# milos-agathon/vulkan-forge

Measured on AMD Instinct MI355X. Metric: Mpix/s terrain shade (grid=4096, 4096x4096), higher is better.
Workload: dtype f32

## Files before the change

### include/vf_hip.h

```cpp
#ifndef VF_HIP_H
#define VF_HIP_H

#include <stddef.h>
#include <stdint.h>

#ifdef __cplusplus
extern "C" {
#endif

#define VF_OK 0
#define VF_ERR_NO_DEVICE (-1)
#define VF_ERR_HIP (-2)
#define VF_ERR_INVALID (-3)
#define VF_ERR_NOMEM (-4)

typedef struct vf_ctx vf_ctx;
typedef struct vf_terrain vf_terrain;

typedef struct vf_device_info {
    char name[256];
    char arch[64];
    int32_t device_ordinal;
    int32_t compute_units;
    int32_t wavefront_size;
// ... 71 lines not shown
int vf_terrain_add_points(vf_terrain *t, const float *xyz, uint32_t n, const float *size_px, const uint8_t *rgba, float default_size,
                          const uint8_t default_rgba[4], int shape, int drape, uint32_t *layer_id);
int vf_terrain_add_lines(vf_terrain *t, const float *xyz, const uint32_t *path_offsets, uint32_t npaths, float width_px,
                         const uint8_t rgba[4], int cap, int drape, uint32_t *layer_id);
int vf_terrain_clear_overlays(vf_terrain *t);
int vf_terrain_add_polygons(vf_terrain *t, const float *xyz, const uint32_t *ring_offsets, uint32_t nrings, const uint32_t *feature_offsets,
                            uint32_t nfeatures, const uint8_t *fill_rgba, const uint8_t default_fill[4], const uint8_t line_rgba[4],
                            float line_width_px, int drape, uint32_t *layer_id);
#define VF_OCCLUSION_DEPTH_BIAS 1e-2f
int vf_terrain_set_layer_occlusion(vf_terrain *t, uint32_t layer_id, int occlude, float depth_bias);
int vf_terrain_set_layer_haze(vf_terrain *t, uint32_t layer_id, int on);
int vf_terrain_layer_haze(vf_terrain *t, uint32_t layer_id, int *on);
#define VF_JOIN_ROUND 0
#define VF_JOIN_NONE 1
int vf_terrain_add_contours(vf_terrain *t, const float *levels, uint32_t nlevels, float width_px, const uint8_t rgba[4], float lift, int join,
                            int occlude, float depth_bias, uint32_t *layer_id, uint32_t *nsegments);
int vf_terrain_height_bounds(vf_terrain *t, float *lo, float *hi);
int vf_terrain_layer_primitive_count(vf_terrain *t, uint32_t layer_id, uint32_t *count);

int vf_terrain_read_rgba(vf_terrain *t, uint8_t *dst, uint32_t y0, uint32_t rows);
int vf_host_alloc(size_t bytes, void **host);
void vf_host_free(void *host);
int vf_terrain_read_png_scanlines(vf_terrain *t, const uint8_t **host_scanlines, size_t *nbytes);
int vf_terrain_read_visibility(vf_terrain *t, uint32_t *dst);

int vf_terrain_enable_timing(vf_terrain *t, int enable);
int vf_terrain_timings(vf_terrain *t, vf_timings *out);
int vf_terrain_frame_times(vf_terrain *t, float *tile_ms, float *period_ms, uint32_t max_frames, uint32_t *count);
int vf_terrain_debug_item_stats(vf_terrain *t, uint32_t *dst, uint32_t max_items, uint32_t *count);
#define VF_BAND_SLOTS 8u
int vf_terrain_debug_band_masks(vf_terrain *t, uint32_t *recs, uint64_t *masks, int32_t *xy, uint32_t max_blocks, uint32_t *count);
int vf_terrain_debug_set_plan_feedback(vf_terrain *t, const uint32_t *tile_ticks, const uint8_t *strips_log2, const uint32_t *piece_ticks,
                                       uint32_t ntiles);
#define VF_PLAN_FIRST        1u
#define VF_PLAN_FRESH        2u
#define VF_PLAN_MOTION_MAP   4u
#define VF_PLAN_DILATE       8u
#define VF_PLAN_QUEUED_AHEAD 16u
#define VF_PLAN_GEOMETRY_REUSED 32u
#define VF_PLAN_TILE_LISTS   64u
int vf_terrain_debug_plan_mode(const vf_terrain *t, uint32_t *mode);
typedef struct vf_tile_list_info { uint32_t built, used, tiles_listed, tiles_fallback, entries, capacity, units_asked, reserved; } vf_tile_list_info;
int vf_terrain_debug_tile_lists(vf_terrain *t, vf_tile_list_info *out);
int vf_terrain_debug_set_tile_list_capacity(vf_terrain *t, uint32_t units);
int vf_terrain_debug_phase_cycles(vf_terrain *t, uint64_t *dst, uint32_t n);

int vf_grid_generate(vf_ctx *ctx, uint32_t nx, uint32_t nz, float dx, float dy,
                     float *xy, float *uv, uint32_t *idx);
int vf_grid_generate_device(vf_ctx *ctx, uint32_t nx, uint32_t nz, float dx, float dy,
                            float *dev_xy, float *dev_uv, uint32_t *dev_idx, void *stream);

int vf_triangle_render(vf_ctx *ctx, uint32_t width, uint32_t height, uint8_t *rgba_host);

typedef struct vf_dem vf_dem;
int vf_dem_create(vf_ctx *ctx, vf_dem **out);
void vf_dem_destroy(vf_dem *d);
int vf_dem_set_heights_f32(vf_dem *d, const float *host, uint32_t w, uint32_t h, float exaggeration);
int vf_dem_set_heights_f64(vf_dem *d, const double *host, uint32_t w, uint32_t h, float exaggeration);
int vf_dem_stats(vf_dem *d, float out[4]);
int vf_dem_percentile_range(vf_dem *d, float *p1, float *p99);
int vf_dem_normalize(vf_dem *d, int mode, float lo, float hi, float eps);
int vf_dem_upload_height(vf_dem *d);
int vf_dem_texture_size(const vf_dem *d, uint32_t *w, uint32_t *h);
int vf_dem_read_patch(vf_dem *d, uint32_t x, uint32_t y, uint32_t w, uint32_t h, float *dst);

int vf_stitch_bands_device(vf_ctx *ctx, const void *dev_gathered, void *dev_image, uint32_t width,
// ... 221 lines not shown
```

### vulkan_forge_amd/cabi.py

```python
from __future__ import annotations

import ctypes as C
import os

import numpy as np

_HERE = os.path.dirname(os.path.abspath(__file__))
DEFAULT_LIB = os.environ.get("VF_HIP_LIB") or os.path.join(_HERE, "libvf_hip.so")

VF_OK, VF_ERR_NO_DEVICE, VF_ERR_HIP, VF_ERR_INVALID, VF_ERR_NOMEM = 0, -1, -2, -3, -4
VF_DRAPE_SIZE_MAX, VF_DRAPE_NEAREST, VF_DRAPE_LINEAR = 16384, 0, 1
VF_DRAPE_MIP_BIAS_MAX, VF_DRAPE_MIP_LEVELS_MAX = 16.0, 15
VF_DRAPE_ANISOTROPY_MAX = 16
VF_SUPERSAMPLE_MAX = 4
VF_PLAN_FIRST, VF_PLAN_FRESH, VF_PLAN_MOTION_MAP, VF_PLAN_DILATE, VF_PLAN_QUEUED_AHEAD = 1, 2, 4, 8, 16
VF_PLAN_TILE_LISTS = 64
VF_PLAN_GEOMETRY_REUSED = 32

SYMBOLS = [
    "vf_last_error", "vf_device_count", "vf_device_query", "vf_ctx_create", "vf_ctx_destroy", "vf_ctx_device_info", "vf_ctx_stream",
    "vf_terrain_create", "vf_terrain_destroy", "vf_terrain_set_uniforms", "vf_terrain_set_height",
    "vf_terrain_set_height_device", "vf_terrain_set_shade_mode", "vf_terrain_set_shade_precision", "vf_terrain_set_raster_groups", "vf_terrain_raster_groups", "vf_terrain_set_shard", "vf_terrain_local_rows", "vf_terrain_set_tile_shard",
    "vf_terrain_local_tiles", "vf_terrain_read_tiles", "vf_tile_layout", "vf_terrain_tile_times", "vf_balance_stripes", "vf_tile_layout_register_map", "vf_terrain_set_output_device",
    "vf_terrain_rgba_device", "vf_terrain_render", "vf_terrain_render_batch", "vf_terrain_render_batch_host", "vf_terrain_sync",
    "vf_terrain_add_points", "vf_terrain_add_lines", "vf_terrain_add_polygons", "vf_terrain_set_layer_occlusion", "vf_terrain_set_layer_haze", "vf_terrain_layer_haze", "vf_terrain_add_contours", "vf_terrain_height_bounds", "vf_terrain_layer_primitive_count", "vf_terrain_clear_overlays", "vf_terrain_read_rgba", "vf_terrain_read_png_scanlines", "vf_terrain_read_visibility",
    "vf_terrain_enable_timing", "vf_terrain_timings", "vf_terrain_frame_times", "vf_terrain_debug_item_stats", "vf_terrain_debug_band_masks", "vf_terrain_debug_set_plan_feedback", "vf_terrain_debug_plan_mode", "vf_terrain_debug_tile_lists", "vf_terrain_debug_set_tile_list_capacity", "vf_terrain_debug_phase_cycles", "vf_grid_generate", "vf_grid_generate_device", "vf_triangle_render",
    "vf_stitch_bands_device", "vf_stitch_tiles_device",
    "vf_dist_available", "vf_dist_version", "vf_dist_unique_id", "vf_dist_comm_init", "vf_dist_comm_destroy", "vf_dist_gather_tiles", "vf_dist_gather_bands", "vf_dist_exchange_bands",
    "vf_terrain_debug_fragment_stage", "vf_host_alloc", "vf_host_free",
    "vf_terrain_gbuffer_device", "vf_terrain_read_gbuffer", "vf_terrain_pick", "vf_terrain_debug_gbuffer_stage",
    "vf_terrain_set_shadows", "vf_terrain_read_shadow_field", "vf_terrain_shadow_field_device", "vf_terrain_debug_shadow_stage",
    "vf_terrain_debug_shadow_scans",
    "vf_terrain_set_ambient", "vf_terrain_read_sky_view_field", "vf_terrain_sky_view_field_device", "vf_terrain_debug_ambient_stage",
    "vf_terrain_debug_ambient_scans",
    "vf_terrain_set_drape", "vf_terrain_set_drape_device", "vf_terrain_clear_drape", "vf_terrain_drape_info", "vf_terrain_debug_drape_stage",
    "vf_terrain_set_drape_mips", "vf_terrain_drape_mip_info", "vf_terrain_read_drape_level", "vf_terrain_debug_drape_mip_build",
    "vf_terrain_set_drape_anisotropy", "vf_terrain_drape_anisotropy",
    "vf_terrain_set_viewshed", "vf_terrain_read_viewshed_field", "vf_terrain_viewshed_field_device", "vf_terrain_viewshed_info",
    "vf_terrain_debug_viewshed_stage", "vf_terrain_debug_viewshed_scans",
    "vf_terrain_set_cumulative_viewshed", "vf_terrain_read_cumulative_viewshed_field", "vf_terrain_cumulative_viewshed_field_device",
    "vf_terrain_cumulative_viewshed_info", "vf_terrain_read_cumulative_viewshed_vertices", "vf_terrain_debug_cumulative_viewshed_batch",
    "vf_terrain_debug_cumulative_viewshed_scans", "vf_terrain_debug_cumulative_viewshed_stage",
    "vf_terrain_set_sun_exposure", "vf_terrain_clear_sun_exposure", "vf_terrain_read_sun_exposure_field", "vf_terrain_sun_exposure_field_device",
    "vf_terrain_sun_exposure_info", "vf_terrain_debug_sun_exposure_batch", "vf_terrain_debug_sun_exposure_scans",
    "vf_terrain_debug_sun_exposure_stage",
    "vf_terrain_create_supersampled", "vf_terrain_supersampling", "vf_terrain_read_samples", "vf_terrain_samples_device",
    "vf_terrain_debug_resolve_stage",
    "vf_terrain_set_haze", "vf_terrain_clear_haze", "vf_terrain_haze_info", "vf_terrain_read_haze_opacity", "vf_terrain_haze_opacity_device",
    "vf_terrain_debug_haze_stage",
    "vf_terrain_set_flood", "vf_terrain_clear_flood", "vf_terrain_read_flood_field", "vf_terrain_flood_field_device", "vf_terrain_flood_info",
    "vf_terrain_read_flood_seeds", "vf_terrain_debug_flood_scans", "vf_terrain_debug_flood_group", "vf_terrain_debug_flood_stage",
    "vf_terrain_set_spill", "vf_terrain_clear_spill", "vf_terrain_read_spill_field", "vf_terrain_spill_field_device", "vf_terrain_read_sink_depth",
    "vf_terrain_spill_info", "vf_terrain_read_spill_seeds", "vf_terrain_debug_spill_scans", "vf_terrain_debug_spill_group",
    "vf_terrain_debug_spill_stage",
    "vf_dem_create", "vf_dem_destroy", "vf_dem_set_heights_f32", "vf_dem_set_heights_f64", "vf_dem_stats",
    "vf_dem_percentile_range", "vf_dem_normalize", "vf_dem_upload_height", "vf_dem_texture_size", "vf_dem_read_patch",
]


# ... 65 lines not shown
    "vf_terrain_set_raster_groups": (_i, [_vp, _i]),
    "vf_terrain_raster_groups": (_i, [_vp, C.POINTER(_i), _vp]),
    "vf_terrain_set_shard": (_i, [_vp, _u32, _u32, _u32]),
    "vf_terrain_local_rows": (_i, [_vp, C.POINTER(_u32)]),
    "vf_terrain_set_tile_shard": (_i, [_vp, _u32, _u32, _u32]),
    "vf_terrain_add_points": (_i, [_vp, _vp, _u32, _vp, _vp, _f, _vp, _i, _i, C.POINTER(_u32)]),
    "vf_terrain_add_lines": (_i, [_vp, _vp, _vp, _u32, _f, _vp, _i, _i, C.POINTER(_u32)]),
    "vf_terrain_add_polygons": (_i, [_vp, _vp, _vp, _u32, _vp, _u32, _vp, _vp, _vp, _f, _i, C.POINTER(_u32)]),
    "vf_terrain_set_layer_occlusion": (_i, [_vp, _u32, _i, _f]),
    "vf_terrain_set_layer_haze": (_i, [_vp, _u32, _i]),
    "vf_terrain_layer_haze": (_i, [_vp, _u32, C.POINTER(C.c_int)]),
    "vf_terrain_add_contours": (_i, [_vp, _vp, _u32, _f, _vp, _f, _i, _i, _f, C.POINTER(_u32), C.POINTER(_u32)]),
    "vf_terrain_height_bounds": (_i, [_vp, C.POINTER(_f), C.POINTER(_f)]),
    "vf_terrain_layer_primitive_count": (_i, [_vp, _u32, C.POINTER(_u32)]),
    "vf_terrain_clear_overlays": (_i, [_vp]),
    "vf_terrain_local_tiles": (_i, [_vp, C.POINTER(_u32)]),
    "vf_terrain_read_tiles": (_i, [_vp, _vp, _u32, _u32]),
    "vf_tile_layout": (_i, [_u32, _u32, _u32, _u32, _u32, _vp, _u32, C.POINTER(_u32)]),
    "vf_terrain_set_output_device": (_i, [_vp, _vp]),
    "vf_terrain_rgba_device": (_i, [_vp, C.POINTER(_vp)]),
    "vf_terrain_render": (_i, [_vp, _vp]),
    "vf_terrain_render_batch": (_i, [_vp, _vp, _u32, _vp, _vp]),
    "vf_terrain_render_batch_host": (_i, [_vp, _vp, _u32, _vp]),
    "vf_terrain_sync": (_i, [_vp]),
    "vf_terrain_read_rgba": (_i, [_vp, _vp, _u32, _u32]),
    "vf_terrain_read_png_scanlines": (_i, [_vp, C.POINTER(_vp), C.POINTER(C.c_size_t)]),
    "vf_terrain_read_visibility": (_i, [_vp, _vp]),
    "vf_terrain_enable_timing": (_i, [_vp, _i]),
    "vf_terrain_timings": (_i, [_vp, C.POINTER(Timings)]),
    "vf_terrain_frame_times": (_i, [_vp, _vp, _vp, _u32, C.POINTER(_u32)]),
    "vf_terrain_debug_item_stats": (_i, [_vp, _vp, _u32, C.POINTER(_u32)]),
    "vf_terrain_debug_band_masks": (_i, [_vp, _vp, _vp, _vp, _u32, C.POINTER(_u32)]),
    "vf_terrain_debug_set_plan_feedback": (_i, [_vp, _vp, _vp, _vp, _u32]),
    "vf_terrain_debug_plan_mode": (_i, [_vp, C.POINTER(_u32)]),
    "vf_terrain_debug_tile_lists": (_i, [_vp, _vp]),
    "vf_terrain_debug_set_tile_list_capacity": (_i, [_vp, _u32]),
    "vf_terrain_debug_phase_cycles": (_i, [_vp, _vp, _u32]),
    "vf_terrain_tile_times": (_i, [_vp, _vp, _u32, C.POINTER(_u32)]),
    "vf_balance_stripes": (_i, [_vp, _u32, _u32, _vp]),
    "vf_tile_layout_register_map": (_i, [_vp, _u32, _u32, _u32, C.POINTER(_u32)]),
    "vf_host_alloc": (_i, [C.c_size_t, C.POINTER(_vp)]),
    "vf_host_free": (None, [_vp]),
    "vf_grid_generate": (_i, [_vp, _u32, _u32, _f, _f, _vp, _vp, _vp]),
    "vf_grid_generate_device": (_i, [_vp, _u32, _u32, _f, _f, _vp, _vp, _vp, _vp]),
    "vf_triangle_render": (_i, [_vp, _u32, _u32, _vp]),
    "vf_stitch_bands_device": (_i, [_vp, _vp, _vp, _u32, _u32, _u32, _u32, _vp]),
    "vf_stitch_tiles_device": (_i, [_vp, _vp, _vp, _u32, _u32, _u32, _u32, _u32, _vp]),
    "vf_dist_available": (_i, []),
    "vf_dist_version": (_i, [C.POINTER(_i)]),
    "vf_dist_unique_id": (_i, [_vp]),
    "vf_dist_comm_init": (_i, [_vp, _vp, _i, _i, C.POINTER(_vp)]),
    "vf_dist_comm_destroy": (None, [_vp]),
    "vf_dist_gather_tiles": (_i, [_vp, _vp, _i, _vp, _u32, _vp]),
    "vf_dist_gather_bands": (_i, [_vp, _vp, _i, _vp, _vp]),
    "vf_dist_exchange_bands": (_i, [_vp, _vp, _i, _vp, _vp]),
    "vf_terrain_debug_fragment_stage": (_i, [_vp, _u32, C.POINTER(FragmentTiming)]),
    "vf_terrain_gbuffer_device": (_i, [_vp, _vp, _vp, _vp, _vp, _vp]),
    "vf_terrain_read_gbuffer": (_i, [_vp, _vp, _vp, _vp, _vp]),
    "vf_terrain_pick": (_i, [_vp, _vp, _u32, _vp]),
    "vf_terrain_debug_gbuffer_stage": (_i, [_vp, _u32, _u32, C.POINTER(_f)]),
    "vf_terrain_set_shadows": (_i, [_vp, _i, _f, _f, _f]),
    "vf_terrain_read_shadow_field": (_i, [_vp, _vp]),
    "vf_terrain_shadow_field_device": (_i, [_vp, _vp, _vp]),
    "vf_terrain_debug_shadow_stage": (_i, [_vp, _u32, C.POINTER(_f)]),
    "vf_terrain_debug_shadow_scans": (_i, [_vp, C.POINTER(_u32)]),
    "vf_terrain_set_ambient": (_i, [_vp, _i, _f, _f, _u32, _vp]),
# ... 768 lines not shown
        a = _u32()
        self._check(self.lib.vf_terrain_drape_anisotropy(self.t, C.byref(a)))
        return a.value

    def enable_timing(self, on=True, stats=True, sampled=False):
        self._check(self.lib.vf_terrain_enable_timing(self.t, (1 if stats else (3 if sampled else 2)) if on else 0))

    def item_stats(self):
        cap = self.timings()["tiles"] + 2048
        out = np.zeros((cap, 4), np.uint32)
        n = _u32()
        self._check(self.lib.vf_terrain_debug_item_stats(self.t, out.ctypes.data, cap, C.byref(n)))
        return out[:n.value]

    def band_masks(self):
        nb = (self.grid - 1 + 7) // 8
        n = nb * nb
        recs, masks, xy = np.zeros((n, 8), np.uint32), np.zeros((n, 8, 2), np.uint64), np.zeros((n, 81, 2), np.int32)
        got = _u32()
        self._check(self.lib.vf_terrain_debug_band_masks(self.t, recs.ctypes.data, masks.ctypes.data, xy.ctypes.data, n, C.byref(got)))
        assert got.value == n
        wide = recs[:, 4:8].copy().view(np.uint64)
        return dict(box=recs[:, 0:2].copy().view(np.int16), flags=recs[:, 2].copy(), count=recs[:, 3].copy(),
                    alive_even=wide[:, 0].copy(), alive_odd=wide[:, 1].copy(), masks=masks, xy=xy)

    def set_plan_feedback(self, tile_ticks, strips_log2=None, piece_ticks=None):
        ticks = np.ascontiguousarray(tile_ticks, dtype=np.uint32).reshape(-1)
        n = len(ticks)
        lg = np.zeros(n, np.uint8) if strips_log2 is None else np.ascontiguousarray(strips_log2, dtype=np.uint8).reshape(n)
        pieces = None if piece_ticks is None else np.ascontiguousarray(piece_ticks, dtype=np.uint32).reshape(n, 64)
        self._check(self.lib.vf_terrain_debug_set_plan_feedback(self.t, ticks.ctypes.data, lg.ctypes.data,
                                                                None if pieces is None else pieces.ctypes.data, n))

    def plan_mode(self, geometry=False):
        m = _u32()
        self._check(self.lib.vf_terrain_debug_plan_mode(self.t, C.byref(m)))
        return m.value if geometry else m.value & ~(VF_PLAN_GEOMETRY_REUSED | VF_PLAN_TILE_LISTS)

    def tile_lists(self):
        w = (_u32 * 8)()
        self._check(self.lib.vf_terrain_debug_tile_lists(self.t, C.addressof(w)))
        names = ("built", "used", "tiles_listed", "tiles_fallback", "entries", "capacity", "units_asked")
        d = dict(zip(names, (int(v) for v in w)))
        d["built"], d["used"] = bool(d["built"]), bool(d["used"])
        return d

    def set_tile_list_capacity(self, units=0xFFFFFFFF):
        self._check(self.lib.vf_terrain_debug_set_tile_list_capacity(self.t, units))

    def geometry_reused(self):
        return bool(self.plan_mode(geometry=True) & VF_PLAN_GEOMETRY_REUSED)

    def tile_stats(self):
        it = self.item_stats()
        out = np.zeros((self.timings()["tiles"], 3), np.uint32)
        tile = it[:, 0] & 0xFFFFF
        np.add.at(out[:, 0], tile, it[:, 1])
        np.maximum.at(out[:, 1], tile, it[:, 2])
        np.maximum.at(out[:, 2], tile, it[:, 3])
        return out

    def phase_cycles(self):
        out = np.zeros(40, np.uint64)
        self._check(self.lib.vf_terrain_debug_phase_cycles(self.t, out.ctypes.data, 40))
        return out

# ... 76 lines not shown
```

### vulkan_forge_amd/csrc/vf_device.h

```cpp
#pragma once
#include <hip/hip_runtime.h>
#include <stdint.h>

#define VF_RESERVE_VGPR(n) asm volatile("" ::: "v" #n)

namespace vf {

constexpr int kBlockCells = 8;
constexpr int kBlockVerts = kBlockCells + 1;
constexpr int kTileW = 64, kTileH = 64;
constexpr uint32_t kSplitQuantumX4 = 7;
#ifndef VF_TILE_MIN_WAVES
#define VF_TILE_MIN_WAVES 5
#endif
#ifndef VF_DIAG_ITEM
#define VF_DIAG_ITEM 0
#endif
constexpr int kDiagItem = VF_DIAG_ITEM;
constexpr int kMaxTileCols = 256;
constexpr int kPhaseSlots = 40;
constexpr int kTileThreads = 1024;
constexpr int kFastExtent = 1 << 24;

constexpr uint32_t F_NEAR = 1u, F_FAR = 2u, F_BAD = 4u, F_NOSNAP = 8u;

struct FrameParams {
    float view[16];
    float proj[16];
    float spacing, exag;
    float h_range, exposure;
    float Lx, Ly, Lz;
    float hw, hh;
    float step;
    uint32_t n, nm1;
    uint32_t nb;
    uint32_t W, H;
    uint32_t ntx, nty;
    uint32_t tw, th;
    uint32_t rank, nranks, band_shift, band_h;
    uint32_t local_rows;
    uint32_t shard_tiles;
    uint32_t skew;
    uint32_t stripe_shift;
    const uint32_t *tile_map;
    const uint8_t *stripe_owner;
    uint32_t clear_rgba;
    uint32_t shade_mode;
    const float *tex;
    float inv2hr;
    uint32_t div_m, div_s;
};
// ... 266 lines not shown
```

### vulkan_forge_amd/csrc/vf_hip.hip

```cpp
#include "../../include/vf_hip.h"
#include "vf_kernels.h"
#include "vf_overlay.h"
#include "vf_gbuffer.h"
#include "vf_shadow.h"
#include "vf_ambient.h"
#include "vf_drape.h"
#include "vf_relight.h"
#include "vf_viewshed.h"
#include "vf_cumulative_viewshed.h"
#include "vf_sun_exposure.h"
#include "vf_resolve.h"
#include "vf_haze.h"
#include "vf_overlay_haze.h"
#include "vf_flood.h"
#include "vf_spill.h"
#include "vf_line_loop.h"

#include <algorithm>
#include <cmath>
#include <vector>
#include <cstddef>
#include <cstdio>
#include <cstring>
#include <cstdlib>
// ... 4075 lines not shown
    *count = (uint32_t)nb;
    return VF_OK;
}

int vf_terrain_debug_set_plan_feedback(vf_terrain *t, const uint32_t *tile_ticks, const uint8_t *strips_log2, const uint32_t *piece_ticks,
                                       uint32_t ntiles)
{
    if (!t || !tile_ticks || !strips_log2) return fail(VF_ERR_INVALID, "NULL argument");
    if (ntiles != t->local_tiles) return fail(VF_ERR_INVALID, "ntiles must be the handle's local tiles");
    for (uint32_t k = 0; k < ntiles; ++k) if (strips_log2[k] > 4u) return fail(VF_ERR_INVALID, "strips_log2 must be 0 .. 4");
    if (t->cursor.frames_since_reset < vf_terrain::kPlanStates)
        return fail(VF_ERR_INVALID, "the handle's first frames are planned from the static estimate: render two frames first");
    for (const auto &S : t->ps) if (!S.slab) return fail(VF_ERR_INVALID, "a plan state has not been used yet: render two frames first");
    VF_HIP_TRY(hipSetDevice(t->ctx->device));
    VF_HIP_TRY(wait_frame(t));
    VF_HIP_TRY(sync_sides(t));
    VF_HIP_TRY(drop_preplan(t));
    VF_HIP_TRY(wait_frame(t));
    VF_HIP_TRY(sync_sides(t));
    if (!ntiles) return VF_OK;
    const size_t all_tiles = (size_t)t->ntx * t->nty;
    std::vector<uint32_t> pieces((size_t)ntiles * 64u, 0u), flags(ntiles);
    if (piece_ticks) std::memcpy(pieces.data(), piece_ticks, pieces.size() * sizeof(uint32_t));
    for (auto &S : t->ps) {
        VF_HIP_TRY(hipMemcpy(S.feedback, tile_ticks, (size_t)ntiles * sizeof(uint32_t), hipMemcpyHostToDevice));
        VF_HIP_TRY(hipMemcpy(S.feedback + all_tiles + 1u, pieces.data(), pieces.size() * sizeof(uint32_t), hipMemcpyHostToDevice));
        VF_HIP_TRY(hipMemcpy(flags.data(), S.background, (size_t)ntiles * sizeof(uint32_t), hipMemcpyDeviceToHost));
        for (uint32_t k = 0; k < ntiles; ++k) flags[k] = (flags[k] & 0xFFu) | ((uint32_t)strips_log2[k] << 8);
        VF_HIP_TRY(hipMemcpy(S.background, flags.data(), (size_t)ntiles * sizeof(uint32_t), hipMemcpyHostToDevice));
    }
    return VF_OK;
}

int vf_terrain_debug_plan_mode(const vf_terrain *t, uint32_t *mode)
{
    if (!t || !mode) return fail(VF_ERR_INVALID, "NULL argument");
    if (!t->rendered) return fail(VF_ERR_INVALID, "nothing rendered yet");
    *mode = t->last_plan_mode;
    return VF_OK;
}

int vf_terrain_debug_tile_lists(vf_terrain *t, vf_tile_list_info *out)
{
    if (!t || !out) return fail(VF_ERR_INVALID, "NULL argument");
    if (!t->rendered) return fail(VF_ERR_INVALID, "nothing rendered yet");
    VF_HIP_TRY(hipSetDevice(t->ctx->device));
    std::memset(out, 0, sizeof *out);
    const vf_terrain::PlanState &S = t->ps[t->last_set];
    out->used = (t->last_plan_mode & VF_PLAN_TILE_LISTS) ? 1u : 0u;
    out->built = lists_valid(t, S) ? 1u : 0u;
    if (!out->built && !out->used) return VF_OK;
    VF_HIP_TRY(hipEventSynchronize(S.listed));
    uint32_t ctl[8];
    VF_HIP_TRY(hipMemcpy(ctl, S.tl_ctl, sizeof ctl, hipMemcpyDeviceToHost));
    out->tiles_listed = ctl[2]; out->tiles_fallback = ctl[3]; out->entries = ctl[4];
    out->capacity = S.tl_cap;
    const unsigned long long asked = (unsigned long long)ctl[0] | ((unsigned long long)ctl[1] << 32);
    out->units_asked = asked > 0xFFFFFFFFull ? 0xFFFFFFFFu : (uint32_t)asked;
    return VF_OK;
}

int vf_terrain_debug_set_tile_list_capacity(vf_terrain *t, uint32_t units)
{
    if (!t) return fail(VF_ERR_INVALID, "NULL argument");
    VF_HIP_TRY(hipSetDevice(t->ctx->device));
    VF_HIP_TRY(wait_frame(t));
// ... 1031 lines not shown
```

### vulkan_forge_amd/csrc/vf_kernels.h

```cpp
#pragma once
#include "vf_device.h"
#include "vf_raster.h"

namespace vf {

__global__ void k_axis_tables(uint32_t n, uint32_t tw, uint32_t th, float *xs, float *sinx, float *cosz,
                              int32_t *txi, int32_t *tyj)
{
    uint32_t i = blockIdx.x * blockDim.x + threadIdx.x;
    if (i >= n) return;
    const float scale = 1.5f;
    const float nm1f = (float)n - 1.0f;
    const float step = (2.0f * scale) / nm1f;
    float x = -scale + (float)i * step;
    float uvc = (float)i / nm1f;
    xs[i] = x;
    sinx[i] = det_sin(x * 1.3f);
    cosz[i] = det_cos(x * 1.1f);
    int tx = (int)floorf(uvc * (float)tw), ty = (int)floorf(uvc * (float)th);
    txi[i] = min(max(tx, 0), (int)tw - 1);
    tyj[i] = min(max(ty, 0), (int)th - 1);
}

__global__ __launch_bounds__(64) void k_height_blocks(uint32_t n, uint32_t nb, uint32_t tw, AxisTables A,
// ... 889 lines not shown
        if ((uint32_t)colbits) atomicOr(&colfin[2 * lane], (uint32_t)colbits);
        if ((uint32_t)(colbits >> 32)) atomicOr(&colfin[2 * lane + 1], (uint32_t)(colbits >> 32));
    }
    return nfinal;
}

struct TilePlace { uint32_t tx; size_t out_base; uint32_t out_stride; };
__device__ __forceinline__ TilePlace tile_rect(const FrameParams &P, uint32_t tile, int32_t &px_lo, int32_t &px_hi, int32_t &py_lo, int32_t &py_hi)
{
    TilePlace tp;
    if (P.shard_tiles) {
        const uint32_t m = P.tile_map[tile];
        tp.tx = m & 0xFFFFu;
        py_lo = (int32_t)((m >> 16) * kTileH);
        tp.out_base = (size_t)tile * (kTileW * kTileH);
        tp.out_stride = kTileW;
    } else {
        tp.tx = tile % P.ntx;
        const uint32_t lty = tile / P.ntx;
        py_lo = (int32_t)global_row(P, lty * kTileH);
        tp.out_base = (size_t)lty * kTileH * P.W + (size_t)tp.tx * kTileW;
        tp.out_stride = P.W;
    }
    px_lo = (int32_t)(tp.tx * kTileW); px_hi = min(px_lo + kTileW, (int32_t)P.W) - 1;
    py_hi = min(py_lo + kTileH, (int32_t)P.H) - 1;
    return tp;
}

constexpr uint32_t kSplitBudget = 2048;
__device__ __forceinline__ uint32_t work_tile(uint32_t code) { return code & 0xFFFFFu; }
__device__ __forceinline__ uint32_t work_part(uint32_t code) { return (code >> 20) & 15u; }
__device__ __forceinline__ uint32_t work_slice(uint32_t code) { return (code >> 27) & 3u; }
__device__ __forceinline__ uint32_t work_lg_slices(uint32_t code) { return (code >> 29) & 3u; }
__device__ __forceinline__ void work_strip(uint32_t code, int32_t &px_lo, int32_t &px_hi)
{
    const uint32_t lg = (code >> 24) & 7u, part = (code >> 20) & 15u;
    const int32_t w = kTileW >> lg;
    const int32_t lo = px_lo + (int32_t)part * w;
    px_hi = min(px_hi, lo + w - 1);
    px_lo = lo;
}


__device__ __forceinline__ uint32_t tile_reach(const FrameParams &P, const PixelBox *__restrict__ row_boxes, const uint32_t *__restrict__ rc_lo,
                                               const uint32_t *__restrict__ rc_hi, uint32_t tcol, int32_t py_lo, int32_t py_hi,
                                               uint32_t *s_hits, uint32_t *s_est)
{
    if (threadIdx.x == 0) { *s_hits = 0; *s_est = 0; }
    __syncthreads();
    uint32_t hits = 0, est = 0;
    for (uint32_t r = threadIdx.x; r < P.nb; r += 256) {
        const PixelBox rr = row_boxes[r];
        const uint32_t lo = rc_lo[tcol * P.nb + r], hi = rc_hi[tcol * P.nb + r];
        if (lo < hi && rr.x0 <= rr.x1 && rr.y1 >= py_lo && rr.y0 <= py_hi) { ++hits; est += hi - lo; }
    }
    for (int o = 32; o > 0; o >>= 1) { hits += __shfl_xor(hits, o); est += __shfl_xor(est, o); }
    if ((threadIdx.x & 63u) == 0 && hits) { atomicAdd(s_hits, hits); atomicAdd(s_est, est); }
    __syncthreads();
    return *s_hits;
}
__device__ __forceinline__ uint32_t static_ticks(uint32_t blocks) { return max(blocks * 25u, 1u); }

__device__ __forceinline__ bool capsule_hits_rect(const float4 &seg, float rad, int32_t px_lo, int32_t px_hi, int32_t py_lo, int32_t py_hi);
__global__ __launch_bounds__(256) void k_plan_estimate(FrameParams P, const PixelBox *__restrict__ row_boxes, const BlockRec *__restrict__ recs,
                                                       const float4 *__restrict__ cap_seg, const float *__restrict__ cap_rad,
                                                       const uint32_t *__restrict__ rc_lo, const uint32_t *__restrict__ rc_hi,
                                                       uint32_t *__restrict__ feedback)
{
    constexpr uint32_t kEstDepth = 24;
    __shared__ uint32_t s_est, s_top[8], s_stop;
    int32_t px_lo, px_hi, py_lo, py_hi;
    const TilePlace tp = tile_rect(P, blockIdx.x, px_lo, px_hi, py_lo, py_hi);
    if (threadIdx.x < 8u) s_top[threadIdx.x] = 0u;
// ... 172 lines not shown
                    }
                }
                {
                    const int32_t tx = (int32_t)tp.tx, ty = (int32_t)(blockIdx.x / P.ntx);
                    for (int32_t dy = -1; dy <= 1; ++dy)
                        for (int32_t dx = -2; dx <= 2; ++dx) {
                            const int32_t x = tx + dx, y = ty + dy;
                            if (x >= 0 && y >= 0 && x < (int32_t)P.ntx && y < (int32_t)P.nty) seen = max(seen, tile_time((uint32_t)y * P.ntx + (uint32_t)x));
                        }
                }
            }
            else if ((seen == 0u || moving) && mean && P.nranks == 1u && !P.shard_tiles) {
                const int32_t tx = (int32_t)tp.tx, ty = (int32_t)(blockIdx.x / P.ntx);
                const int32_t reach = seen ? 1 : 2;
                for (int32_t dy = -reach; dy <= reach; ++dy)
                    for (int32_t dx = -reach; dx <= reach; ++dx) {
                        const int32_t x = tx + dx, y = ty + dy;
                        if (x >= 0 && y >= 0 && x < (int32_t)P.ntx && y < (int32_t)P.nty) seen = max(seen, tile_time((uint32_t)y * P.ntx + (uint32_t)x));
                    }
            }
            const uint32_t weight = seen ? seen : static_ticks(s_est);
            uint32_t lg = 0, lgs = 0;
            if (mean && px_hi - px_lo + 1 == kTileW) {
                const uint32_t q = seen / mean;
                lg = q >= 16u ? 4u : q >= 8u ? 3u : q >= 4u ? 2u : q >= 2u ? 1u : 0u;
                while (lg + lgs && atomicAdd(split_budget, (1u << (lg + lgs)) - 1u) + (1u << (lg + lgs)) - 1u > kSplitBudget) {
                    atomicSub(split_budget, (1u << (lg + lgs)) - 1u);
                    if (lgs) --lgs; else --lg;
                }
            }
            const uint32_t cut = lg | (lgs << 4);
            const bool same_cut = own_time && seen == tile_time(blockIdx.x) && seen != 0u && ((last_flags[blockIdx.x] >> 8) & 0x3Fu) == cut;
            const uint32_t *piece_time = last_blocks + (size_t)P.ntx * P.nty + 1u + (size_t)blockIdx.x * 64u;
            flags_out[blockIdx.x] = cut << 8;
            const uint32_t parts = 1u << lg, slices = 1u << lgs;
            const uint32_t at = atomicAdd(work_count, parts * slices);
            for (uint32_t p = 0; p < parts; ++p)
                for (uint32_t sl = 0; sl < slices; ++sl)
                    work[at + p * slices + sl] = make_uint2(blockIdx.x | (p << 20) | (lg << 24) | (sl << 27) | (lgs << 29),
                                                            same_cut ? max(piece_time[p * slices + sl], 1u) : weight >> (lg + lgs));
        }
        return;
    }
    if (threadIdx.x == 0) flags_out[blockIdx.x] = 1u;
}

__global__ __launch_bounds__(256) void k_clear(FrameParams P, const uint32_t *__restrict__ background, uint32_t *__restrict__ rgba,
                                               uint32_t *__restrict__ vis_out, uint32_t *__restrict__ stats, uint32_t nstats,
                                               uint32_t *__restrict__ seg_count)
{
    if (blockIdx.x == 0 && threadIdx.x == 0) *seg_count = 0u;
    if (stats) for (uint32_t k = blockIdx.x * 256u + threadIdx.x; k < nstats; k += gridDim.x * 256u) stats[k] = 0u;
    if ((background[blockIdx.x] & 1u) == 0u) return;
    int32_t px_lo, px_hi, py_lo, py_hi;
    const TilePlace tp = tile_rect(P, blockIdx.x, px_lo, px_hi, py_lo, py_hi);
    const int32_t w = px_hi - px_lo + 1, h = py_hi - py_lo + 1;
    if (w == kTileW && (tp.out_stride & 3u) == 0u && (tp.out_base & 3u) == 0u && (reinterpret_cast<uintptr_t>(rgba) & 15u) == 0u &&
        (!vis_out || (reinterpret_cast<uintptr_t>(vis_out) & 15u) == 0u)) {
        const uint4 c4 = make_uint4(P.clear_rgba, P.clear_rgba, P.clear_rgba, P.clear_rgba), z4 = make_uint4(0u, 0u, 0u, 0u);
        for (int32_t k = threadIdx.x; k < (kTileW / 4) * h; k += 256) {
            const int32_t ly = k / (kTileW / 4), q = k - ly * (kTileW / 4);
            const size_t o = tp.out_base + (size_t)ly * tp.out_stride + 4u * (uint32_t)q;
            *reinterpret_cast<uint4 *>(rgba + o) = c4;
            if (vis_out) *reinterpret_cast<uint4 *>(vis_out + o) = z4;
        }
        return;
    }
// ... 11 lines not shown
{
    constexpr uint32_t kKeys = 1024, kT = 256;
    __shared__ uint32_t s_hist[kKeys];
    __shared__ uint32_t s_kr[4096];
    __shared__ uint32_t s_wsum[kT / 64];
    const uint32_t n = *work_count, tid = threadIdx.x, lane = tid & 63u, wave = tid >> 6;
    for (uint32_t k = tid; k < ntiles; k += kT) last_blocks[k] = 0u;
    for (uint32_t k = tid; k < nlocal; k += kT) background[k] = flags_new[k];
    for (uint32_t base = 0; base < n; base += 4096) {
        const uint32_t m = min(4096u, n - base);
        for (uint32_t k = tid; k < kKeys; k += kT) s_hist[k] = 0u;
        __syncthreads();
#pragma unroll 1
        for (uint32_t k = tid; k < m; k += kT) {
            const uint32_t f = (__float_as_uint((float)max(work[base + k].y, 1u)) >> 18) - (127u << 5);
            const uint32_t key = (kKeys - 1u) - min(f, kKeys - 1u);
            s_kr[k] = key | (atomicAdd(&s_hist[key], 1u) << 10);
        }
        __syncthreads();
        const uint32_t a0 = s_hist[4u * tid], a1 = s_hist[4u * tid + 1u], a2 = s_hist[4u * tid + 2u], a3 = s_hist[4u * tid + 3u];
        const uint32_t mine = a0 + a1 + a2 + a3;
        const uint32_t inc = wave_scan_add(mine);
        if (lane == 63u) s_wsum[wave] = inc;
        __syncthreads();
        uint32_t before = 0;
#pragma unroll
        for (uint32_t w = 0; w < kT / 64; ++w) before += w < wave ? s_wsum[w] : 0u;
        const uint32_t first = before + inc - mine;
        s_hist[4u * tid] = first; s_hist[4u * tid + 1u] = first + a0; s_hist[4u * tid + 2u] = first + a0 + a1; s_hist[4u * tid + 3u] = first + a0 + a1 + a2;
        __syncthreads();
#pragma unroll 1
        for (uint32_t k = tid; k < m; k += kT) {
            const uint32_t kr = s_kr[k];
            sorted[base + s_hist[kr & (kKeys - 1u)] + (kr >> 10)] = work[base + k];
        }
        __syncthreads();
    }
}

#ifdef VF_PHASE_PROF
struct PhaseClock {
    uint64_t acc[20], last;
    __device__ __forceinline__ void start() { for (int k = 0; k < 20; ++k) acc[k] = 0; last = __builtin_readcyclecounter(); }
    __device__ __forceinline__ void tick(int p) { const uint64_t now = __builtin_readcyclecounter(); acc[p] += now - last; last = now; }
};
#define VF_PH_INIT PhaseClock PH; PH.start();
#define VF_PH(p) PH.tick(p);
#define VF_PH_ARG , PhaseClock &PH
#define VF_PH_PASS , PH
#else
#define VF_PH_INIT
#define VF_PH(p)
#define VF_PH_ARG
#define VF_PH_PASS
#endif
struct TileLists { const uint4 *ent; const uint4 *hdr; };
namespace tile {
constexpr int kWaves = kTileThreads / 64;
constexpr int kNV = kBlockVerts * kBlockVerts;
constexpr uint32_t kChunk = 4096;
constexpr int kMaxSteps = 128;
constexpr int kHitWords = 16;
constexpr int kRescanEvery = 1;
constexpr int kBlockPrims = 2 * kBlockCells * kBlockCells;
constexpr uint32_t kWideLines = 28, kBalGain = 2;
struct WaveLds {
    int2 xy[kWaves][kNV];
// ... 325 lines not shown
    WaveLds &s_wave = *reinterpret_cast<WaveLds *>(s_overlay);
    int2 (&sXY)[kWaves][kNV] = s_wave.xy;
    uint32_t (&sS)[kWaves][kBlockPrims] = s_wave.surv;
    Lds L;
    L.vis = s_vis; L.hit = reinterpret_cast<unsigned long long (*)[kHitWords]>(s_overlay);
    L.xy = s_wave.xy; L.surv = s_wave.surv;
    L.list = s_list; L.cnt = s_cnt; L.words = s_words; L.pending = s_pending; L.firstid = s_firstid; L.allrows = s_allrows; L.rc = s_rc;
    L.colfin = s_colfin; L.rowfin = s_rowfin; L.colfin4 = s_colfin4; L.rowfin4 = s_rowfin4; L.part = s_part; L.rows = s_rows;
    L.next = &s_next; L.lock = &s_lock; L.done = &s_done; L.frontier = &s_frontier; L.published = &s_published; L.blocks = &s_blocks; L.redo = &s_redo;
    L.per = s_per;

    const uint32_t tid = threadIdx.x, lane = tid & 63u;
    const uint32_t wave = (uint32_t)__builtin_amdgcn_readfirstlane((int)(tid >> 6));
    VF_PH_INIT
    VF_RC(RasterCounts RC = {};)
    uint32_t redo_at = blockIdx.x;
    if (COMPLETE && redo_at >= *redo_count) return;
    for (int k = tid; k < kLutFloats; k += kTileThreads) s_lut[k] = lut_linear[k];
    for (int k = tid; k < 256; k += kTileThreads) s_thr[k] = thresh[k];
    if (tid <= 64u) { const uint32_t per = tid ? 64u / tid : 64u; s_per[tid] = per | (((65536u + per - 1u) / per) << 7) | ((64u / per) << 24); }
    const ShadeTables S = { s_lut, s_thr };
    const uint32_t nwork = *work_count;
    uint32_t pulled = 0;
    if (!COMPLETE) {
        if (tid == 0) s_item = atomicAdd(work_count + 2, 1u);
        __syncthreads();
        pulled = (uint32_t)__builtin_amdgcn_readfirstlane((int)s_item);
        if (pulled >= nwork) return;
    }
    for (;;) {
    VF_PH(12)
    const uint32_t item_idx = COMPLETE ? redo[redo_at] : pulled;
    const uint64_t t_start = __builtin_amdgcn_s_memrealtime();
    const uint32_t item = work[item_idx].x;
    const uint32_t tile = work_tile(item);
    TileCtx T;
    T.vis = s_vis; T.colfin = s_colfin; T.rowfin = s_rowfin; T.colfin4 = s_colfin4; T.rowfin4 = s_rowfin4;
    const TilePlace tp = tile_rect(P, tile, T.px_lo, T.px_hi, T.py_lo, T.py_hi);
    const uint32_t tcol = tp.tx;
    static_assert(kTileH == 64, "the set-up pass folds rows of 64 pixels");
    const uint32_t band_slot = (uint32_t)__builtin_amdgcn_readfirstlane((int)(((uint32_t)T.py_lo >> 6) & ((uint32_t)kBandSlots - 1u)));
    const int32_t tile_x0 = T.px_lo;
    work_strip(item, T.px_lo, T.px_hi);
    const uint32_t tile_pixels = (uint32_t)(T.px_hi - T.px_lo + 1) * (uint32_t)(T.py_hi - T.py_lo + 1);
    const uint64_t row_full = ~0ull >> (63 - (T.px_hi - T.px_lo));

    for (int k = tid; k < kTileW * kTileH; k += kTileThreads) s_vis[k] = 0u;
    for (int k = tid; k < kTileW * 2; k += kTileThreads) s_colfin[k] = 0u;
    for (int k = tid; k < kTileH * 2; k += kTileThreads) s_rowfin[k] = 0u;
    if (tid < kTileW / 4 * 2) { s_colfin4[tid] = 0u; s_rowfin4[tid] = 0u; }
    if (tid < 16) s_rows[tid] = 0ull;
    if (tid == 0) {
        s_done = 0; s_blocks = 0; s_redo = 0;
        uint4 th = make_uint4(0u, 0xFFFFFFFFu, 0u, 0u);
        if (TL.hdr) th = TL.hdr[tile];
        s_tl[0] = th.x; s_tl[1] = th.y; s_tl[2] = th.z; s_tl[3] = th.w;
    }
    __syncthreads();
    VF_PH(13)
    const bool listed = lds_peek(&s_tl[1]) != 0xFFFFFFFFu;
    uint32_t nrows_total;
    if (listed) { const uint32_t n = lds_peek(&s_tl[1]), rows = lds_peek(&s_tl[2]); nrows_total = n ? (rows & 0xFFFFu) - (rows >> 16) + 1u : 0u; }
    else nrows_total = list_block_rows(P, L, T, row_boxes, rc_lo, rc_hi, tcol, tid, lane, wave VF_PH_PASS);
    VF_PH(8)
    uint32_t dbg_loop = 0;
    const uint32_t hit_words = (P.nb + 63u) / 64u;
    for (uint32_t cursor = 0; cursor < nrows_total;) {
        if (tid == 0) { s_next = 0; s_lock = 0; s_frontier = 0; s_published = 0; }
        uint32_t nsteps, nlist;
        if (lds_peek(&s_tl[1]) != 0xFFFFFFFFu) {
            const uint32_t e0 = (uint32_t)__builtin_amdgcn_readfirstlane((int)lds_peek(&s_tl[0])), o0 = (uint32_t)__builtin_amdgcn_readfirstlane((int)lds_peek(&s_tl[3]));
            const uint32_t row_hi = (uint32_t)__builtin_amdgcn_readfirstlane((int)lds_peek(&s_tl[2])) & 0xFFFFu;
            take_listed_rows<GROUPS>(P, L, T, TL.ent + e0, reinterpret_cast<const uint32_t *>(TL.ent + o0), cap_seg, cap_rad, ((item >> 24) & 7u) != 0u, row_hi, cursor, nrows_total,
                                     tid, lane, wave, nsteps, nlist VF_PH_PASS);
        } else {
        const uint32_t nrowsteps = min((uint32_t)kMaxSteps, nrows_total - cursor);
// ... 180 lines not shown
            if (GROUPS) __builtin_amdgcn_s_setprio(3);
            uint32_t fr = lds_peek(&s_frontier);
            while (fr < nsteps && lds_peek(&s_pending[fr]) == 0u) ++fr;
            const uint32_t pub = lds_peek(&s_published);
            if (fr > pub && (fr - pub >= (uint32_t)kRescanEvery || fr == nsteps)) {
                const int32_t sw = T.px_hi - T.px_lo + 1, sh = T.py_hi - T.py_lo + 1;
                const uint32_t nfinal = sw <= 16 ? rescan_strip(s_vis, s_colfin, s_rowfin, lane, s_firstid[fr - 1], sw, sh)
                                                 : rescan_open_rows(s_vis, s_colfin, s_rowfin, lane, s_firstid[fr - 1], row_full, sh);
                if constexpr (GROUPS) {
                    __builtin_amdgcn_wave_barrier();
                    refresh_fin4(s_colfin, s_rowfin, s_colfin4, s_rowfin4, lane);
                }
                if (lane == 0) { s_published = fr; if (nfinal >= tile_pixels) { s_done = 1u; atomicOr(&s_next, 0x40000000u); } }
            }
            if (lane == 0) { s_frontier = fr; __threadfence_block(); atomicExch(&s_lock, 0u); }
            __builtin_amdgcn_s_setprio(0);
            VF_PH(5)
        }
        VF_PH(1)
        __builtin_amdgcn_s_setprio(0);
        if (lane == 0 && my_blocks) atomicAdd(&s_blocks, my_blocks);
        __syncthreads();
        if (kDiagItem == 1) dbg_loop += (uint32_t)(__builtin_amdgcn_s_memrealtime() - dbg_t0);
        if (s_done) break;
        const uint32_t all = publish_chunk_masks<GROUPS>(L, nsteps, lane, wave);
        VF_PH(6)
        if (all >= tile_pixels) break;
    }
    __syncthreads();
    VF_PH(6)
    if (stats && tid == 0) {
        atomicAdd(&stats[0], s_blocks);
        stats[4 + 4 * item_idx] = item;
        stats[5 + 4 * item_idx] = kDiagItem == 1 ? dbg_loop : kDiagItem == 2 ? work[item_idx].y : kDiagItem == 3 ? (uint32_t)t_start : s_blocks;
        stats[6 + 4 * item_idx] = (uint32_t)(__builtin_amdgcn_s_memrealtime() - t_start);
    }
    shade_item<WRITE_VIS, COMPLETE, FAST>(P, V, S, L, T, tp, tile_x0, rgba, vis_out, tid);
    VF_PH(7)
    if (tid == 0) {
        const uint32_t ticks = (uint32_t)(__builtin_amdgcn_s_memrealtime() - t_start);
        atomicAdd(&last_blocks[tile], max(ticks, 1u));
        if (!COMPLETE)
            last_blocks[(size_t)P.ntx * P.nty + 1u + (size_t)tile * 64u + work_part(item)] = max(ticks, 1u);
        if (stats) stats[7 + 4 * item_idx] = ticks;
        if (!COMPLETE && s_redo) redo[atomicAdd(redo_count, 1u)] = item_idx;
    }
    __syncthreads();
    if constexpr (COMPLETE) {
        redo_at += gridDim.x;
        if (redo_at >= *redo_count) break;
    }
    else {
        if (tid == 0) s_item = atomicAdd(work_count + 2, 1u);
        __syncthreads();
        pulled = (uint32_t)__builtin_amdgcn_readfirstlane((int)s_item);
        if (pulled >= nwork) break;
    }
    }
#ifdef VF_PHASE_PROF
    if (stats) {
        unsigned long long *ph = reinterpret_cast<unsigned long long *>(stats + 4 + 4 * ((size_t)P.ntx * P.nty + kSplitBudget));
        if (lane == 0) {
            for (int p = 0; p < 8; ++p) atomicAdd(&ph[p], (unsigned long long)PH.acc[p]);
            for (int p = 8; p < 16; ++p) atomicAdd(&ph[8 + p], (unsigned long long)PH.acc[p]);
            atomicAdd(&ph[30], (unsigned long long)PH.acc[16]); atomicAdd(&ph[31], (unsigned long long)PH.acc[17]);
            atomicAdd(&ph[32], (unsigned long long)PH.acc[18]); atomicAdd(&ph[33], (unsigned long long)PH.acc[19]);
            atomicAdd(&ph[8], (unsigned long long)RC.nsurv); atomicAdd(&ph[9], (unsigned long long)RC.iters);
// ... 395 lines not shown
```

Measured before the change: 27270.

## Adapt tile strip boundaries from per-piece timings to balance split work items

When a tile is split into 2 or 4 column strips, the planner now moves the strip edges each frame based on the measured time of neighbouring pieces. Edges are packed into the per-tile flags and decoded into the work item's second word during sorting. The shade kernel reads its column range from that word instead of splitting evenly. The aim is to reduce load imbalance between pieces of the same tile, at the cost of extra planning logic and a repurposed work word. Debug APIs to read and set the edges are added.

```diff
diff --git a/include/vf_hip.h b/include/vf_hip.h
--- a/include/vf_hip.h
+++ b/include/vf_hip.h
@@ -127,6 +127,8 @@
 int vf_terrain_debug_band_masks(vf_terrain *t, uint32_t *recs, uint64_t *masks, int32_t *xy, uint32_t max_blocks, uint32_t *count);
 int vf_terrain_debug_set_plan_feedback(vf_terrain *t, const uint32_t *tile_ticks, const uint8_t *strips_log2, const uint32_t *piece_ticks,
                                        uint32_t ntiles);
+int vf_terrain_debug_strip_edges(vf_terrain *t, uint32_t *edges, uint32_t ntiles);
+int vf_terrain_debug_set_strip_edges(vf_terrain *t, const uint32_t *edges, uint32_t ntiles);
 #define VF_PLAN_FIRST        1u
 #define VF_PLAN_FRESH        2u
 #define VF_PLAN_MOTION_MAP   4u
diff --git a/vulkan_forge_amd/cabi.py b/vulkan_forge_amd/cabi.py
--- a/vulkan_forge_amd/cabi.py
+++ b/vulkan_forge_amd/cabi.py
@@ -24,7 +24,7 @@
     "vf_terrain_local_tiles", "vf_terrain_read_tiles", "vf_tile_layout", "vf_terrain_tile_times", "vf_balance_stripes", "vf_tile_layout_register_map", "vf_terrain_set_output_device",
     "vf_terrain_rgba_device", "vf_terrain_render", "vf_terrain_render_batch", "vf_terrain_render_batch_host", "vf_terrain_sync",
     "vf_terrain_add_points", "vf_terrain_add_lines", "vf_terrain_add_polygons", "vf_terrain_set_layer_occlusion", "vf_terrain_set_layer_haze", "vf_terrain_layer_haze", "vf_terrain_add_contours", "vf_terrain_height_bounds", "vf_terrain_layer_primitive_count", "vf_terrain_clear_overlays", "vf_terrain_read_rgba", "vf_terrain_read_png_scanlines", "vf_terrain_read_visibility",
-    "vf_terrain_enable_timing", "vf_terrain_timings", "vf_terrain_frame_times", "vf_terrain_debug_item_stats", "vf_terrain_debug_band_masks", "vf_terrain_debug_set_plan_feedback", "vf_terrain_debug_plan_mode", "vf_terrain_debug_tile_lists", "vf_terrain_debug_set_tile_list_capacity", "vf_terrain_debug_phase_cycles", "vf_grid_generate", "vf_grid_generate_device", "vf_triangle_render",
+    "vf_terrain_enable_timing", "vf_terrain_timings", "vf_terrain_frame_times", "vf_terrain_debug_item_stats", "vf_terrain_debug_band_masks", "vf_terrain_debug_set_plan_feedback", "vf_terrain_debug_strip_edges", "vf_terrain_debug_set_strip_edges", "vf_terrain_debug_plan_mode", "vf_terrain_debug_tile_lists", "vf_terrain_debug_set_tile_list_capacity", "vf_terrain_debug_phase_cycles", "vf_grid_generate", "vf_grid_generate_device", "vf_triangle_render",
     "vf_stitch_bands_device", "vf_stitch_tiles_device",
     "vf_dist_available", "vf_dist_version", "vf_dist_unique_id", "vf_dist_comm_init", "vf_dist_comm_destroy", "vf_dist_gather_tiles", "vf_dist_gather_bands", "vf_dist_exchange_bands",
     "vf_terrain_debug_fragment_stage", "vf_host_alloc", "vf_host_free",
@@ -156,6 +156,8 @@
     "vf_terrain_debug_item_stats": (_i, [_vp, _vp, _u32, C.POINTER(_u32)]),
     "vf_terrain_debug_band_masks": (_i, [_vp, _vp, _vp, _vp, _u32, C.POINTER(_u32)]),
     "vf_terrain_debug_set_plan_feedback": (_i, [_vp, _vp, _vp, _vp, _u32]),
+    "vf_terrain_debug_strip_edges": (_i, [_vp, _vp, _u32]),
+    "vf_terrain_debug_set_strip_edges": (_i, [_vp, _vp, _u32]),
     "vf_terrain_debug_plan_mode": (_i, [_vp, C.POINTER(_u32)]),
     "vf_terrain_debug_tile_lists": (_i, [_vp, _vp]),
     "vf_terrain_debug_set_tile_list_capacity": (_i, [_vp, _u32]),
@@ -990,6 +992,17 @@
         self._check(self.lib.vf_terrain_debug_set_plan_feedback(self.t, ticks.ctypes.data, lg.ctypes.data,
                                                                 None if pieces is None else pieces.ctypes.data, n))
 
+    def strip_edges(self):
+        n = _u32()
+        self._check(self.lib.vf_terrain_local_tiles(self.t, C.byref(n)))
+        out = np.zeros(n.value, np.uint32)
+        self._check(self.lib.vf_terrain_debug_strip_edges(self.t, out.ctypes.data, n.value))
+        return out
+
+    def set_strip_edges(self, edges):
+        e = np.ascontiguousarray(edges, dtype=np.uint32).reshape(-1)
+        self._check(self.lib.vf_terrain_debug_set_strip_edges(self.t, e.ctypes.data, len(e)))
+
     def plan_mode(self, geometry=False):
         m = _u32()
         self._check(self.lib.vf_terrain_debug_plan_mode(self.t, C.byref(m)))
diff --git a/vulkan_forge_amd/csrc/vf_device.h b/vulkan_forge_amd/csrc/vf_device.h
--- a/vulkan_forge_amd/csrc/vf_device.h
+++ b/vulkan_forge_amd/csrc/vf_device.h
@@ -17,6 +17,15 @@
 #define VF_DIAG_ITEM 0
 #endif
 constexpr int kDiagItem = VF_DIAG_ITEM;
+#ifndef VF_EDGE_GAIN_INV
+#define VF_EDGE_GAIN_INV 4
+#endif
+#ifndef VF_EDGE_CAP
+#define VF_EDGE_CAP 4
+#endif
+#ifndef VF_STRIP_EDGES
+#define VF_STRIP_EDGES 1
+#endif
 constexpr int kMaxTileCols = 256;
 constexpr int kPhaseSlots = 40;
 constexpr int kTileThreads = 1024;
diff --git a/vulkan_forge_amd/csrc/vf_hip.hip b/vulkan_forge_amd/csrc/vf_hip.hip
--- a/vulkan_forge_amd/csrc/vf_hip.hip
+++ b/vulkan_forge_amd/csrc/vf_hip.hip
@@ -4131,6 +4131,46 @@
     return VF_OK;
 }
 
+int vf_terrain_debug_strip_edges(vf_terrain *t, uint32_t *edges, uint32_t ntiles)
+{
+    if (!t || !edges) return fail(VF_ERR_INVALID, "NULL argument");
+    if (ntiles != t->local_tiles) return fail(VF_ERR_INVALID, "ntiles must be the handle's local tiles");
+    if (!t->rendered) return fail(VF_ERR_INVALID, "nothing rendered");
+    const vf_terrain::PlanState &S = t->ps[t->last_set];
+    if (!S.slab) return fail(VF_ERR_INVALID, "nothing rendered");
+    VF_HIP_TRY(hipSetDevice(t->ctx->device));
+    VF_HIP_TRY(wait_frame(t));
+    VF_HIP_TRY(sync_sides(t));
+    if (!ntiles) return VF_OK;
+    VF_HIP_TRY(hipMemcpy(edges, S.background, (size_t)ntiles * sizeof(uint32_t), hipMemcpyDeviceToHost));
+    for (uint32_t k = 0; k < ntiles; ++k) edges[k] >>= kEdgeShift;
+    return VF_OK;
+}
+
+int vf_terrain_debug_set_strip_edges(vf_terrain *t, const uint32_t *edges, uint32_t ntiles)
+{
+    if (!t || !edges) return fail(VF_ERR_INVALID, "NULL argument");
+    if (ntiles != t->local_tiles) return fail(VF_ERR_INVALID, "ntiles must be the handle's local tiles");
+    for (uint32_t k = 0; k < ntiles; ++k) if (edges[k] >> (32u - kEdgeShift)) return fail(VF_ERR_INVALID, "edges are three 6-bit columns");
+    if (t->cursor.frames_since_reset < vf_terrain::kPlanStates)
+        return fail(VF_ERR_INVALID, "the handle's first frames are planned from the static estimate: render two frames first");
+    for (const auto &S : t->ps) if (!S.slab) return fail(VF_ERR_INVALID, "a plan state has not been used yet: render two frames first");
+    VF_HIP_TRY(hipSetDevice(t->ctx->device));
+    VF_HIP_TRY(wait_frame(t));
+    VF_HIP_TRY(sync_sides(t));
+    VF_HIP_TRY(drop_preplan(t));
+    VF_HIP_TRY(wait_frame(t));
+    VF_HIP_TRY(sync_sides(t));
+    if (!ntiles) return VF_OK;
+    std::vector<uint32_t> flags(ntiles);
+    for (auto &S : t->ps) {
+        VF_HIP_TRY(hipMemcpy(flags.data(), S.background, (size_t)ntiles * sizeof(uint32_t), hipMemcpyDeviceToHost));
+        for (uint32_t k = 0; k < ntiles; ++k) flags[k] = (flags[k] & ((1u << kEdgeShift) - 1u)) | (edges[k] << kEdgeShift);
+        VF_HIP_TRY(hipMemcpy(S.background, flags.data(), (size_t)ntiles * sizeof(uint32_t), hipMemcpyHostToDevice));
+    }
+    return VF_OK;
+}
+
 int vf_terrain_debug_plan_mode(const vf_terrain *t, uint32_t *mode)
 {
     if (!t || !mode) return fail(VF_ERR_INVALID, "NULL argument");
diff --git a/vulkan_forge_amd/csrc/vf_kernels.h b/vulkan_forge_amd/csrc/vf_kernels.h
--- a/vulkan_forge_amd/csrc/vf_kernels.h
+++ b/vulkan_forge_amd/csrc/vf_kernels.h
@@ -945,13 +945,57 @@
 __device__ __forceinline__ uint32_t work_part(uint32_t code) { return (code >> 20) & 15u; }
 __device__ __forceinline__ uint32_t work_slice(uint32_t code) { return (code >> 27) & 3u; }
 __device__ __forceinline__ uint32_t work_lg_slices(uint32_t code) { return (code >> 29) & 3u; }
-__device__ __forceinline__ void work_strip(uint32_t code, int32_t &px_lo, int32_t &px_hi)
-{
-    const uint32_t lg = (code >> 24) & 7u, part = (code >> 20) & 15u;
-    const int32_t w = kTileW >> lg;
-    const int32_t lo = px_lo + (int32_t)part * w;
-    px_hi = min(px_hi, lo + w - 1);
-    px_lo = lo;
+constexpr uint32_t kEdgeShift = 14;
+constexpr int32_t kStripFloor = 8;
+constexpr uint32_t kEdgeDeadInv = 32, kEdgeGainInv = VF_EDGE_GAIN_INV, kEdgeCap = VF_EDGE_CAP;
+constexpr bool kStripEdges = VF_STRIP_EDGES != 0;
+__device__ __forceinline__ void strip_bounds(uint32_t lg, uint32_t edges, int32_t b[5])
+{
+    const int32_t parts = 1 << lg;
+    b[0] = 0;
+    bool ok = edges != 0u;
+    for (int32_t p = 1; p < parts; ++p) { b[p] = (int32_t)((edges >> (6 * (p - 1))) & 63u); ok = ok && b[p] - b[p - 1] >= kStripFloor; }
+    b[parts] = kTileW;
+    ok = ok && b[parts] - b[parts - 1] >= kStripFloor;
+    if (!ok) for (int32_t p = 1; p < parts; ++p) b[p] = p * (kTileW >> lg);
+}
+__device__ __forceinline__ uint32_t strip_edges_update(uint32_t lg, uint32_t recorded, const uint32_t *piece_time)
+{
+    int32_t b[5], n[5];
+    strip_bounds(lg, recorded, b);
+    const int32_t parts = 1 << lg;
+    n[0] = 0; n[parts] = kTileW;
+    for (int32_t p = 1; p < parts; ++p) {
+        const unsigned long long a = piece_time[p - 1], c = piece_time[p], sum = a + c, diff = a > c ? a - c : c - a;
+        n[p] = b[p];
+        if (a && c && diff * kEdgeDeadInv > sum) {
+            const unsigned long long den = sum * kEdgeGainInv;
+            const int32_t m = (int32_t)min((diff * (unsigned long long)(b[p + 1] - b[p - 1]) + den / 2ull) / den, (unsigned long long)kEdgeCap);
+            n[p] = a > c ? b[p] - m : b[p] + m;
+        }
+    }
+    for (int32_t p = 1; p < parts; ++p) n[p] = max(n[p], n[p - 1] + kStripFloor);
+    for (int32_t p = parts - 1; p >= 1; --p) n[p] = min(n[p], n[p + 1] - kStripFloor);
+    uint32_t e = 0; bool even = true;
+    for (int32_t p = 1; p < parts; ++p) { e |= (uint32_t)n[p] << (6 * (p - 1)); even = even && n[p] == p * (kTileW >> lg); }
+    return even ? 0u : e;
+}
+__device__ __forceinline__ uint32_t work_columns(uint32_t code, uint32_t flags)
+{
+    const uint32_t lg = (code >> 24) & 7u, part = (code >> 20) & 15u, edges = flags >> kEdgeShift;
+    if ((lg == 1u || lg == 2u) && edges) {
+        int32_t b[5];
+        strip_bounds(lg, edges, b);
+        return (uint32_t)b[part] | ((uint32_t)(b[part + 1] - 1) << 6);
+    }
+    const uint32_t w = (uint32_t)kTileW >> lg;
+    return (part * w) | ((part * w + w - 1u) << 6);
+}
+__device__ __forceinline__ void work_strip(uint32_t cols, int32_t &px_lo, int32_t &px_hi)
+{
+    const int32_t x0 = px_lo;
+    px_hi = min(px_hi, x0 + (int32_t)((cols >> 6) & 63u));
+    px_lo = x0 + (int32_t)(cols & 63u);
 }
 
 
@@ -1190,7 +1234,10 @@
             const uint32_t cut = lg | (lgs << 4);
             const bool same_cut = own_time && seen == tile_time(blockIdx.x) && seen != 0u && ((last_flags[blockIdx.x] >> 8) & 0x3Fu) == cut;
             const uint32_t *piece_time = last_blocks + (size_t)P.ntx * P.nty + 1u + (size_t)blockIdx.x * 64u;
-            flags_out[blockIdx.x] = cut << 8;
+            uint32_t edges = 0;
+            if (kStripEdges && (lg == 1u || lg == 2u) && lgs == 0u && same_cut)
+                edges = strip_edges_update(lg, last_flags[blockIdx.x] >> kEdgeShift, piece_time);
+            flags_out[blockIdx.x] = (cut << 8) | (edges << kEdgeShift);
             const uint32_t parts = 1u << lg, slices = 1u << lgs;
             const uint32_t at = atomicAdd(work_count, parts * slices);
             for (uint32_t p = 0; p < parts; ++p)
@@ -1268,7 +1315,8 @@
 #pragma unroll 1
         for (uint32_t k = tid; k < m; k += kT) {
             const uint32_t kr = s_kr[k];
-            sorted[base + s_hist[kr & (kKeys - 1u)] + (kr >> 10)] = work[base + k];
+            const uint2 w = work[base + k];
+            sorted[base + s_hist[kr & (kKeys - 1u)] + (kr >> 10)] = make_uint2(w.x, work_columns(w.x, flags_new[work_tile(w.x)]) | (min(w.y, 0xFFFFFu) << 12));
         }
         __syncthreads();
     }
@@ -1660,7 +1708,8 @@
     VF_PH(12)
     const uint32_t item_idx = COMPLETE ? redo[redo_at] : pulled;
     const uint64_t t_start = __builtin_amdgcn_s_memrealtime();
-    const uint32_t item = work[item_idx].x;
+    const uint2 item_words = work[item_idx];
+    const uint32_t item = item_words.x, cols = item_words.y;
     const uint32_t tile = work_tile(item);
     TileCtx T;
     T.vis = s_vis; T.colfin = s_colfin; T.rowfin = s_rowfin; T.colfin4 = s_colfin4; T.rowfin4 = s_rowfin4;
@@ -1669,7 +1718,7 @@
     static_assert(kTileH == 64, "the set-up pass folds rows of 64 pixels");
     const uint32_t band_slot = (uint32_t)__builtin_amdgcn_readfirstlane((int)(((uint32_t)T.py_lo >> 6) & ((uint32_t)kBandSlots - 1u)));
     const int32_t tile_x0 = T.px_lo;
-    work_strip(item, T.px_lo, T.px_hi);
+    work_strip(cols, T.px_lo, T.px_hi);
     const uint32_t tile_pixels = (uint32_t)(T.px_hi - T.px_lo + 1) * (uint32_t)(T.py_hi - T.py_lo + 1);
     const uint64_t row_full = ~0ull >> (63 - (T.px_hi - T.px_lo));
 
@@ -1916,7 +1965,7 @@
     if (stats && tid == 0) {
         atomicAdd(&stats[0], s_blocks);
         stats[4 + 4 * item_idx] = item;
-        stats[5 + 4 * item_idx] = kDiagItem == 1 ? dbg_loop : kDiagItem == 2 ? work[item_idx].y : kDiagItem == 3 ? (uint32_t)t_start : s_blocks;
+        stats[5 + 4 * item_idx] = kDiagItem == 1 ? dbg_loop : kDiagItem == 2 ? cols >> 12 : kDiagItem == 3 ? (uint32_t)t_start : s_blocks;
         stats[6 + 4 * item_idx] = (uint32_t)(__builtin_amdgcn_s_memrealtime() - t_start);
     }
     shade_item<WRITE_VIS, COMPLETE, FAST>(P, V, S, L, T, tp, tile_x0, rgba, vis_out, tid);
```

Result: no change. 27480 (median of 6 runs) (+0.8%).
